# opas-lab/olearning-sim

Hardware: AMD Instinct MI355X
Metric: virtual clients/sec (simulated FL rounds, FedAvg CNN) (higher is better)
Workload: dtype bfloat16; 1 GPU; model=resnet18, preset=resnet-10k, clients_total=1250, clients_per_gpu=1250, local_steps=2, local_batch=16, num_classes=100, parallelism=dp1, global_batch=20000

## Files before the change

olearning_sim_amd/engine/local_train.py:

```python

from __future__ import annotations

from typing import Dict, Optional

import torch

from ..models.base import ClientBatchedModel, Params
from ..ops import fused
from .client_manager import FlatParams, replicate_params
from .data import SyntheticFederatedData


class LocalTrainer:
    def __init__(self, model: ClientBatchedModel, master: FlatParams,
                 data: SyntheticFederatedData, lr: float, prox_mu: float,
                 local_steps: int, batch_size: int, dtype: torch.dtype,
                 report_loss: bool = True):
        self.report_loss = report_loss
        self.model = model
        self.master = master
        self.data = data
        self.lr = lr
        self.prox_mu = prox_mu
        self.local_steps = local_steps
        self.batch_size = batch_size
        self.dtype = dtype
        self._cast_flat: Optional[torch.Tensor] = None

    def begin_round(self) -> None:
        self._cast_flat = self.master.flat.to(self.dtype)

    def _cast_params(self) -> Params:
        assert self._cast_flat is not None, "begin_round() not called"
        return self.master.views_of(self._cast_flat)

    def train_chunk(self, client_ids: torch.Tensor, weights: torch.Tensor,
                    round_idx: int, delta_flat: torch.Tensor,
                    wsum: Optional[float] = None) -> Dict[str, float]:
        C = int(client_ids.numel())
        cast = self._cast_params()
        params = replicate_params(cast, C)
        plist = list(params.values())
        glist = [cast[k] for k in params]
        last_loss = 0.0
        for step in range(self.local_steps):
            x, y = self.data.batch(client_ids, round_idx, step,
                                   self.batch_size, self.dtype)
            loss = self.model.loss(params, x, y)
            grads = torch.autograd.grad(loss * C, plist, allow_unused=True)
            with torch.no_grad():
                live = [(p, g) for p, g in zip(plist, grads) if g is not None]
                fused.fused_sgd_update(
                    [p for p, _ in live], [g for _, g in live],
                    lr=self.lr, mu=self.prox_mu,
                    global_params=[cast[k] for k, g in
                                   zip(params, grads) if g is not None])
            if self.report_loss and step == self.local_steps - 1:
                last_loss = float(loss.detach())
            del grads
        with torch.no_grad():
            delta_views = list(self.master.views_of(delta_flat).values())
            fused.weighted_delta_accum(
                delta_views, [p.detach() for p in plist], glist, weights,
                wsum=wsum if wsum is not None else float(weights.sum()))
        return {"loss": last_loss, "clients": C}
```

olearning_sim_amd/models/resnet.py:

```python

from __future__ import annotations

from typing import Optional

import torch

from .base import (ClientBatchedModel, Params, binit, kaiming,
                   blinear, bconv2d)

_STAGES = (64, 128, 256, 512)
_GN_GROUPS = 8


class ResNet18(ClientBatchedModel):
    name = "resnet18"
    num_classes = 100
    act_elems_per_sample = 1_600_000
    input_shape = (3, 32, 32)

    def __init__(self, num_classes: int = 100, in_ch: int = 3,
                 width_mult: float = 1.0):
        self.num_classes = num_classes
        self.in_ch = in_ch
        self.widths = [int(w * width_mult) for w in _STAGES]
        self.input_shape = (in_ch, 32, 32)

    def init_global(self, device="cpu", dtype=torch.float32,
                    generator: Optional[torch.Generator] = None) -> Params:
        g = generator
        p: Params = {}

        def conv(name, oc, ic, k):
            p[f"{name}.w"] = kaiming((oc, ic, k, k), ic * k * k, device, dtype, g)

        def gn(name, ch):
            p[f"{name}.g"] = torch.ones(ch, device=device, dtype=dtype)
            p[f"{name}.b"] = torch.zeros(ch, device=device, dtype=dtype)

        w = self.widths
        conv("stem", w[0], self.in_ch, 3)
        gn("stem.gn", w[0])
        in_c = w[0]
        for s, out_c in enumerate(w):
            for blk in range(2):
                pre = f"s{s}.b{blk}"
                ic = in_c if blk == 0 else out_c
                conv(f"{pre}.c1", out_c, ic, 3)
                gn(f"{pre}.gn1", out_c)
                conv(f"{pre}.c2", out_c, out_c, 3)
                gn(f"{pre}.gn2", out_c)
                if blk == 0 and (ic != out_c or s > 0):
                    conv(f"{pre}.down", out_c, ic, 1)
                    gn(f"{pre}.gndown", out_c)
            in_c = out_c
        p["fc.w"] = binit((w[3], self.num_classes), w[3], device, dtype, g)
        p["fc.b"] = binit((self.num_classes,), w[3], device, dtype, g)
        return p

    def _block(self, params: Params, x: torch.Tensor, C: int, pre: str,
               stride: int, has_down: bool) -> torch.Tensor:
        from ..ops.fused import groupnorm_act
        h = bconv2d(x, params[f"{pre}.c1.w"], C, stride=stride, padding=1)
        h = groupnorm_act(h, C, _GN_GROUPS, params[f"{pre}.gn1.g"],
                          params[f"{pre}.gn1.b"], relu=True)
        h = bconv2d(h, params[f"{pre}.c2.w"], C, stride=1, padding=1)
        if has_down:
            sc = bconv2d(x, params[f"{pre}.down.w"], C, stride=stride)
            sc = groupnorm_act(sc, C, _GN_GROUPS, params[f"{pre}.gndown.g"],
                               params[f"{pre}.gndown.b"])
        else:
            sc = x
        return groupnorm_act(h, C, _GN_GROUPS, params[f"{pre}.gn2.g"],
                             params[f"{pre}.gn2.b"], res=sc, relu=True)

    def _block_cbf(self, params: Params, x: torch.Tensor, x_pad, C: int,
                   pre: str, stride: int, has_down: bool,
                   pad_out: bool = True):
        from ..ops.conv import conv3x3_gn_relu, client_conv1x1
        from ..ops.fused import groupnorm_act
        h, h_pad = conv3x3_gn_relu(x, x_pad, params[f"{pre}.c1.w"], stride,
                                   C, _GN_GROUPS, params[f"{pre}.gn1.g"],
                                   params[f"{pre}.gn1.b"])
        if has_down:
            sc = client_conv1x1(x, params[f"{pre}.down.w"], stride,
                                x_pad=x_pad)
            sc = groupnorm_act(sc, C, _GN_GROUPS, params[f"{pre}.gndown.g"],
                               params[f"{pre}.gndown.b"])
            sc_pad = None
        else:
            sc, sc_pad = x, x_pad
        return conv3x3_gn_relu(h, h_pad, params[f"{pre}.c2.w"], 1, C,
                               _GN_GROUPS, params[f"{pre}.gn2.g"],
                               params[f"{pre}.gn2.b"], res=sc,
                               res_pad=sc_pad, pad_out=pad_out)

    def forward_cbf(self, params: Params, x: torch.Tensor) -> torch.Tensor:
        from ..ops.conv import client_conv3x3
        from ..ops.fused import groupnorm_relu_pad
        C, B = x.shape[0], x.shape[1]
        h = x.permute(0, 2, 1, 3, 4).contiguous()
        h = client_conv3x3(h, params["stem.w"], 1)
        h, h_pad = groupnorm_relu_pad(h, C, _GN_GROUPS, params["stem.gn.g"],
                                      params["stem.gn.b"])
        for s in range(4):
            stride = 1 if s == 0 else 2
            h, h_pad = self._block_cbf(params, h, h_pad, C, f"s{s}.b0",
                                       stride, s > 0)
            h, h_pad = self._block_cbf(params, h, h_pad, C, f"s{s}.b1", 1,
                                       False, pad_out=s < 3)
        h = h.mean(dim=(3, 4)).permute(0, 2, 1)
        return blinear(h, params["fc.w"], params["fc.b"])

    def forward(self, params: Params, x: torch.Tensor) -> torch.Tensor:
        from ..ops.fused import groupnorm_act
        import os
        if x.is_cuda and x.dtype == torch.bfloat16 and \
                os.environ.get("OLSIM_CONV", "custom") == "custom":
            from ..ops.fused import hip_ops_available
            if hip_ops_available():
                return self.forward_cbf(params, x)
        C, B = x.shape[0], x.shape[1]
        h = x.permute(1, 0, 2, 3, 4).reshape(B, C * self.in_ch, 32, 32)
        h = bconv2d(h, params["stem.w"], C, stride=1, padding=1)
        h = groupnorm_act(h, C, _GN_GROUPS, params["stem.gn.g"],
                          params["stem.gn.b"], relu=True)
        for s in range(4):
            stride = 1 if s == 0 else 2
            has_down = s > 0
            h = self._block(params, h, C, f"s{s}.b0", stride, has_down)
            h = self._block(params, h, C, f"s{s}.b1", 1, False)
        h = h.mean(dim=(2, 3)).reshape(B, C, self.widths[3]).permute(1, 0, 2)
        return blinear(h, params["fc.w"], params["fc.b"])
```

olearning_sim_amd/ops/build.py:

```python

from __future__ import annotations

import os
import shutil
import sys


def build(verbose: bool = True) -> str:
    os.environ.setdefault("PYTORCH_ROCM_ARCH", "gfx950")
    here = os.path.dirname(os.path.abspath(__file__))
    csrc = os.path.join(here, "csrc")
    build_dir = os.path.join(here, "_build")
    os.makedirs(build_dir, exist_ok=True)
    sources = [os.path.join(csrc, f) for f in
               ("bindings.cpp", "fused_update.hip", "aggregate.hip",
                "cross_entropy.hip", "groupnorm.hip", "client_conv.hip",
                "client_conv2.hip", "client_conv5.hip", "pool2x2.hip", "transpose.hip", "layernorm.hip", "pad2d.hip",
               "replicate.hip")]
    from torch.utils.cpp_extension import load
    mod_path = load(
        name="olsim_hip_ops",
        sources=sources,
        extra_cflags=["-O3"],
        extra_cuda_cflags=["-O3"],
        build_directory=build_dir,
        is_python_module=False,
        verbose=verbose,
    )
    built = os.path.join(build_dir, "olsim_hip_ops.so")
    target = os.path.join(here, "_hip_ops.so")
    if os.path.exists(built):
        shutil.copy2(built, target)
    return target


if __name__ == "__main__":
    path = build()
    print(f"built: {path}", file=sys.stderr)
```

olearning_sim_amd/ops/conv.py:

```python

from __future__ import annotations

import torch
import torch.nn.functional as F

from .fused import load_hip_ops


def _cpu_conv3x3(x: torch.Tensor, w: torch.Tensor, stride: int) -> torch.Tensor:
    C, IC, B, H, W = x.shape
    OC = w.shape[1]
    xg = x.permute(2, 0, 1, 3, 4).reshape(B, C * IC, H, W)
    wf = w.reshape(C * OC, IC, 3, 3)
    y = F.conv2d(xg, wf, stride=stride, padding=1, groups=C)
    OH, OW = y.shape[-2:]
    return y.reshape(B, C, OC, OH, OW).permute(1, 2, 0, 3, 4).contiguous()


class _Conv3x3Fn(torch.autograd.Function):
    @staticmethod
    def forward(ctx, x, w, stride):
        ops = load_hip_ops(required=True)
        y = ops.conv3x3_fwd(x, w, stride)
        ctx.save_for_backward(x, w)
        ctx.stride = stride
        return y

    @staticmethod
    def backward(ctx, dy):
        x, w = ctx.saved_tensors
        ops = load_hip_ops(required=True)
        dy = dy.contiguous()
        dx = dw = None
        if ctx.needs_input_grad[0]:
            dx = ops.conv3x3_dgrad(dy, w, x.shape[3], x.shape[4], ctx.stride)
        if ctx.needs_input_grad[1]:
            dw = ops.conv3x3_wgrad(x, dy, ctx.stride)
        return dx, dw, None


def _pad(x: torch.Tensor, pad: int) -> torch.Tensor:
    import os
    if (x.is_cuda and x.dtype == torch.bfloat16 and x.shape[-1] % 2 == 0
            and os.environ.get("OLSIM_PAD", "") != "torch"):
        ops = load_hip_ops()
        if ops is not None:
            return ops.pad2d(x.contiguous(), pad)
    return F.pad(x, (pad, pad, pad, pad))


class _Conv3x3PadFn(torch.autograd.Function):

    @staticmethod
    def forward(ctx, x, w, stride):
        ops = load_hip_ops(required=True)
        x_pad = _pad(x, 1)
        y = ops.conv3x3_fwd_p(x_pad, w, stride)
        ctx.save_for_backward(x_pad, w)
        ctx.stride = stride
        return y

    @staticmethod
    def backward(ctx, dy):
        x_pad, w = ctx.saved_tensors
        ops = load_hip_ops(required=True)
        dy = dy.contiguous()
        dx = dw = None
        H, W = x_pad.shape[3] - 2, x_pad.shape[4] - 2
        if ctx.needs_input_grad[0]:
            dy_pad = _pad(dy, 1)
            dx = ops.conv3x3_dgrad_p(dy_pad, w, H, W, ctx.stride)
        if ctx.needs_input_grad[1]:
            dw = ops.conv3x3_wgrad_p(x_pad, dy, ctx.stride)
        return dx, dw, None


class _Conv3x3GnPadFn(torch.autograd.Function):

    @staticmethod
    def forward(ctx, x, x_pad, w, res, res_pad, gamma, beta, clients,
                groups, eps, stride, pad_out):
        from .fused import _interior, _res_arg
        ops = load_hip_ops(required=True)
        h = ops.conv3x3_fwd_p(x_pad, w, stride)
        y, mask, mean, rstd = ops.groupnorm_fwd_pad(
            h, _res_arg(h, res, res_pad), gamma, beta, clients, groups, eps,
            pad_out)
        ctx.save_for_backward(x_pad, w, h, mask, mean, rstd, gamma)
        ctx.meta = (clients, groups, res is not None, stride)
        ctx.set_materialize_grads(False)
        if not pad_out:
            return y, None
        ctx.mark_non_differentiable(y)
        return _interior(y), y

    @staticmethod
    def backward(ctx, dy, _dy_pad):
        x_pad, w, h, mask, mean, rstd, gamma = ctx.saved_tensors
        clients, groups, has_res, stride = ctx.meta
        if dy is None:
            return (None,) * 12
        ops = load_hip_ops(required=True)
        need_dx = ctx.needs_input_grad[0]
        dh, dh_pad, dres, dgamma, dbeta = ops.groupnorm_bwd_pad(
            h, mask, dy, mean, rstd, gamma, clients, groups, has_res,
            need_dx)
        H, W = x_pad.shape[3] - 2, x_pad.shape[4] - 2
        dx = dw = None
        if need_dx:
            dx = ops.conv3x3_dgrad_p(dh_pad, w, H, W, stride)
        if ctx.needs_input_grad[2]:
            dw = ops.conv3x3_wgrad_p(x_pad, dh, stride)
        return (dx, None, dw, dres if has_res else None, None,
                dgamma.to(gamma.dtype), dbeta.to(gamma.dtype),
                None, None, None, None, None)


def conv3x3_gn_relu(x: torch.Tensor, x_pad, w: torch.Tensor, stride: int,
                    clients: int, groups: int, gamma: torch.Tensor,
                    beta: torch.Tensor, res=None, res_pad=None,
                    pad_out: bool = True, eps: float = 1e-5):
    from .fused import gn_pad_shape_ok, groupnorm_act
    if x.is_cuda and x.dtype == torch.bfloat16:
        ops = load_hip_ops(required=True)
        OH = (x.shape[3] + stride - 1) // stride
        OW = (x.shape[4] + stride - 1) // stride
        if _v6_ok(ops, x, w, stride) and gn_pad_shape_ok(w.shape[1], groups,
                                                         OH, OW):
            if x_pad is None:
                x_pad = _pad(x, 1)
            return _Conv3x3GnPadFn.apply(
                x, x_pad, w.contiguous(), res, res_pad, gamma.contiguous(),
                beta.contiguous(), clients, groups, eps, stride, pad_out)
    h = client_conv3x3(x, w, stride)
    return groupnorm_act(h, clients, groups, gamma, beta, res=res,
                         relu=True, eps=eps), None


def _v6_ok(ops, x: torch.Tensor, w: torch.Tensor, stride: int) -> bool:
    import os
    if os.environ.get("OLSIM_CONV_V", "") == "5":
        return False
    C, IC, B, H, W = x.shape
    return bool(ops.conv3x3_v6_ok(IC, w.shape[1], B, H, W, stride))


def client_conv3x3(x: torch.Tensor, w: torch.Tensor,
                   stride: int = 1) -> torch.Tensor:
    if x.is_cuda and x.dtype == torch.bfloat16:
        ops = load_hip_ops(required=True)
        if _v6_ok(ops, x, w, stride):
            return _Conv3x3PadFn.apply(x.contiguous(), w.contiguous(), stride)
        return _Conv3x3Fn.apply(x.contiguous(), w.contiguous(), stride)
    return _cpu_conv3x3(x, w, stride)



_NTAB_CACHE: dict = {}


def _ntab(B: int, OH: int, OW: int, H: int, W: int,
          device: torch.device) -> torch.Tensor:
    key = (B, OH, OW, H, W, str(device))
    t = _NTAB_CACHE.get(key)
    if t is None:
        n = torch.arange(B * OH * OW, dtype=torch.int64)
        b, q = n // (OH * OW), n % (OH * OW)
        t = (b * H * W + (q // OW) * W + (q % OW)).to(torch.int32).to(device)
        if len(_NTAB_CACHE) < 64:
            _NTAB_CACHE[key] = t
    return t


def _cpu_conv5x5(x, w, b, relu):
    C, IC, B, H, W = x.shape
    OC = w.shape[1]
    xg = x.permute(2, 0, 1, 3, 4).reshape(B, C * IC, H, W)
    y = F.conv2d(xg, w.reshape(C * OC, IC, 5, 5), b.reshape(C * OC),
                 groups=C)
    OH, OW = y.shape[-2:]
    y = y.reshape(B, C, OC, OH, OW).permute(1, 2, 0, 3, 4).contiguous()
    return F.relu(y) if relu else y


class _Conv5x5Fn(torch.autograd.Function):

    @staticmethod
    def forward(ctx, x, w, b, relu):
        ops = load_hip_ops(required=True)
        C, IC, B, H, W = x.shape
        nt = _ntab(B, H - 4, W - 4, H, W, x.device)
        y = ops.conv5x5_fwd(x, w, b, nt, relu)
        ctx.save_for_backward(x, w, y)
# ... 115 lines not shown
```

olearning_sim_amd/ops/csrc/bindings.cpp:

```cpp

#include <torch/extension.h>
#include <ATen/cuda/CUDAContext.h>
#include <hip/hip_runtime.h>

#include "ols_ops.h"

namespace {

int dtype_code(const at::Tensor& t) {
  switch (t.scalar_type()) {
    case at::kFloat: return 0;
    case at::kBFloat16: return 1;
    case at::kHalf: return 2;
    default:
      TORCH_CHECK(false, "olsim_hip: unsupported dtype ", t.scalar_type());
  }
}

void fused_sgd_update_flat(at::Tensor buf, at::Tensor grad,
                           at::Tensor global_flat, at::Tensor offsets,
                           int64_t clients, double lr, double mu) {
  TORCH_CHECK(buf.is_cuda() && buf.is_contiguous(), "buf must be GPU+contig");
  TORCH_CHECK(grad.sizes() == buf.sizes() && grad.scalar_type() == buf.scalar_type());
  const bool prox = mu != 0.0 && global_flat.numel() > 0;
// ... 187 lines not shown
                  d.B, d.H, d.W, (int)stride,
                  at::cuda::getCurrentCUDAStream().stream());
  return y;
}

at::Tensor conv3x3_dgrad(at::Tensor dy, at::Tensor w, int64_t H, int64_t W,
                         int64_t stride) {
  const ConvDims d = conv_dims(3, {}, 0, dy, 0, w, H, W, stride);
  auto dx = at::empty({d.C, d.IC, d.B, d.H, d.W}, dy.options());
  ols_conv3x3_dgrad(dy.data_ptr(), w.data_ptr(), dx.data_ptr(), d.C, d.IC,
                    d.OC, d.B, d.H, d.W, (int)stride,
                    at::cuda::getCurrentCUDAStream().stream());
  return dx;
}

at::Tensor conv3x3_wgrad(at::Tensor x, at::Tensor dy, int64_t stride) {
  const ConvDims d = conv_dims(3, x, 0, dy, 0, {}, 0, 0, stride);
  auto dw = at::empty({d.C, d.OC, d.IC, 3, 3}, x.options());
  ols_conv3x3_wgrad(x.data_ptr(), dy.data_ptr(), dw.data_ptr(), d.C, d.IC,
                    d.OC, d.B, d.H, d.W, (int)stride,
                    at::cuda::getCurrentCUDAStream().stream());
  return dw;
}


bool conv3x3_v6_ok(int64_t IC, int64_t OC, int64_t B, int64_t H, int64_t W,
                   int64_t stride) {
  return ols_conv3x3_v6_ok((int)IC, (int)OC, (int)B, (int)H, (int)W,
                           (int)stride) != 0;
}

std::string conv3x3_route(std::string dir, int64_t IC, int64_t OC, int64_t B,
                          int64_t H, int64_t W, int64_t stride) {
  int d = dir == "fwd" ? 0 : dir == "dgrad" ? 1 : dir == "wgrad" ? 2 : -1;
  TORCH_CHECK(d >= 0, "conv3x3_route: dir must be fwd, dgrad or wgrad");
  TORCH_CHECK(stride == 1 || stride == 2, "conv3x3_route: stride 1 or 2");
  return ols_conv3x3_route(d, (int)IC, (int)OC, (int)B, (int)H, (int)W,
                           (int)stride);
}

std::string conv3x3_staging(std::string dir, int64_t IC, int64_t OC,
                            int64_t B, int64_t H, int64_t W, int64_t stride) {
  int d = dir == "fwd" ? 0 : dir == "dgrad" ? 1 : dir == "wgrad" ? 2 : -1;
  TORCH_CHECK(d >= 0, "conv3x3_staging: dir must be fwd, dgrad or wgrad");
  TORCH_CHECK(stride == 1 || stride == 2, "conv3x3_staging: stride 1 or 2");
  return ols_conv3x3_staging(d, (int)IC, (int)OC, (int)B, (int)H, (int)W,
                             (int)stride);
}

void check_v6(const ConvDims& d, int64_t stride) {
  TORCH_CHECK(ols_conv3x3_v6_ok(d.IC, d.OC, d.B, d.H, d.W, (int)stride),
              "shape unsupported by the v6 conv path");
}

at::Tensor conv3x3_fwd_p(at::Tensor xp, at::Tensor w, int64_t stride) {
  const ConvDims d = conv_dims(3, xp, 1, {}, 0, w, 0, 0, stride);
  check_v6(d, stride);
  auto y = at::empty({d.C, d.OC, d.B, d.OH, d.OW}, xp.options());
  ols_conv3x3_fwd_p(xp.data_ptr(), w.data_ptr(), y.data_ptr(), d.C, d.IC,
                    d.OC, d.B, d.H, d.W, (int)stride,
                    at::cuda::getCurrentCUDAStream().stream());
  return y;
}

at::Tensor conv3x3_dgrad_p(at::Tensor dyp, at::Tensor w, int64_t H, int64_t W,
                           int64_t stride) {
  const ConvDims d = conv_dims(3, {}, 0, dyp, 1, w, H, W, stride);
  check_v6(d, stride);
  auto dx = at::empty({d.C, d.IC, d.B, d.H, d.W}, dyp.options());
  ols_conv3x3_dgrad_p(dyp.data_ptr(), w.data_ptr(), dx.data_ptr(), d.C, d.IC,
                      d.OC, d.B, d.H, d.W, (int)stride,
                      at::cuda::getCurrentCUDAStream().stream());
  return dx;
}

at::Tensor conv3x3_wgrad_p(at::Tensor xp, at::Tensor dy, int64_t stride) {
  const ConvDims d = conv_dims(3, xp, 1, dy, 0, {}, 0, 0, stride);
  check_v6(d, stride);
  auto dw = at::empty({d.C, d.OC, d.IC, 3, 3}, xp.options());
  ols_conv3x3_wgrad_p(xp.data_ptr(), dy.data_ptr(), dw.data_ptr(), d.C, d.IC,
                      d.OC, d.B, d.H, d.W, (int)stride,
                      at::cuda::getCurrentCUDAStream().stream());
  return dw;
}


std::string conv5x5_route(std::string dir, int64_t IC, int64_t OC, int64_t H,
                          int64_t W) {
  int d = dir == "fwd" ? 0 : dir == "dgrad" ? 1 : dir == "wgrad" ? 2 : -1;
  TORCH_CHECK(d >= 0, "conv5x5_route: dir must be fwd, dgrad or wgrad");
  int r = ols_conv5x5_route(d, (int)IC, (int)OC, (int)H, (int)W);
  return r == 0 ? "direct" : r == 1 ? "mfma" : "two_stage";
}

void check_ntab(const at::Tensor& ntab, const at::Tensor& on, int64_t n) {
  TORCH_CHECK(ntab.is_cuda() && ntab.device() == on.device() &&
                  ntab.scalar_type() == at::kInt && ntab.is_contiguous() &&
                  ntab.numel() == n,
              "conv5x5: ntab must be ", n, " contiguous int32 on the GPU");
}

at::Tensor conv5x5_fwd(at::Tensor x, at::Tensor w, at::Tensor bias,
                       at::Tensor ntab, bool relu) {
  const ConvDims d = conv_dims(5, x, 0, {}, 0, w, 0, 0, 1);
  TORCH_CHECK(d.OC <= 16);
  check_ntab(ntab, x, (int64_t)d.B * d.OH * d.OW);
  TORCH_CHECK(bias.is_cuda() && bias.scalar_type() == at::kBFloat16 &&
              bias.numel() == (int64_t)d.C * d.OC);
  auto y = at::empty({d.C, d.OC, d.B, d.OH, d.OW}, x.options());
  ols_conv5x5_fwd(x.data_ptr(), w.data_ptr(), bias.contiguous().data_ptr(),
                  y.data_ptr(), ntab.data_ptr<int>(), d.C, d.IC, d.OC, d.B,
                  d.H, d.W, relu ? 1 : 0,
                  at::cuda::getCurrentCUDAStream().stream());
  return y;
}

at::Tensor conv5x5_dgrad(at::Tensor dyp, at::Tensor w, at::Tensor ntab,
                         int64_t H, int64_t W) {
  const ConvDims d = conv_dims(5, {}, 0, dyp, 4, w, H, W, 1);
  TORCH_CHECK(d.IC <= 16);
  check_ntab(ntab, dyp, (int64_t)d.B * d.H * d.W);
  auto dx = at::empty({d.C, d.IC, d.B, d.H, d.W}, dyp.options());
  ols_conv5x5_dgrad(dyp.data_ptr(), w.data_ptr(), dx.data_ptr(),
                    ntab.data_ptr<int>(), d.C, d.IC, d.OC, d.B, d.H, d.W,
                    at::cuda::getCurrentCUDAStream().stream());
  return dx;
}

at::Tensor conv5x5_wgrad(at::Tensor x, at::Tensor dy, at::Tensor ntab) {
  const ConvDims d = conv_dims(5, x, 0, dy, 0, {}, 0, 0, 1);
  const int64_t nq = (int64_t)d.B * d.OH * d.OW;
  TORCH_CHECK(d.OC <= 16 && nq % 32 == 0);
  check_ntab(ntab, x, nq);
  auto dw = at::empty({d.C, d.OC, d.IC, 5, 5}, x.options());
  at::Tensor part;
  float* partp = nullptr;
  if (ols_conv5x5_route(2, d.IC, d.OC, d.H, d.W) == 2) {
    part = at::empty({(int64_t)d.C * d.B * d.OC * d.IC * 25},
                     x.options().dtype(at::kFloat));
    partp = part.data_ptr<float>();
  }
  ols_conv5x5_wgrad(x.data_ptr(), dy.data_ptr(), dw.data_ptr(), partp,
                    ntab.data_ptr<int>(), d.C, d.IC, d.OC, d.B, d.H, d.W,
                    at::cuda::getCurrentCUDAStream().stream());
  return dw;
}


std::tuple<at::Tensor, at::Tensor> pool2x2_fwd(at::Tensor x) {
  TORCH_CHECK(x.is_cuda() && x.is_contiguous() && x.dim() >= 2);
  int H = x.size(-2), W = x.size(-1);
  TORCH_CHECK(H % 2 == 0 && W % 2 == 0);
  int64_t planes = x.numel() / ((int64_t)H * W);
  auto sizes = x.sizes().vec();
  sizes[sizes.size() - 2] = H / 2;
  sizes[sizes.size() - 1] = W / 2;
  auto y = at::empty(sizes, x.options());
  auto arg = at::empty(sizes, x.options().dtype(at::kByte));
  int dt = x.scalar_type() == at::kBFloat16 ? 1 : 0;
  ols_pool2x2_fwd(x.data_ptr(), y.data_ptr(),
                  (unsigned char*)arg.data_ptr(), planes, H / 2, W / 2, dt,
                  at::cuda::getCurrentCUDAStream().stream());
  return {y, arg};
}

at::Tensor pool2x2_bwd(at::Tensor dy, at::Tensor arg) {
// ... 195 lines not shown
              y.scalar_type() == at::kLong);
  int64_t rows = y.numel(), batch = x.size(0), n = x.size(1);
  TORCH_CHECK(rows % batch == 0);
  auto out = at::empty({rows, n}, x.options().dtype(at::kBFloat16));
  ols_synth_batch(x.data_ptr<float>(), y.data_ptr<int64_t>(),
                  out.data_ptr(), rows, batch, n, (float)s, (float)t,
                  at::cuda::getCurrentCUDAStream().stream());
  return out;
}


at::Tensor relu_mask(at::Tensor dy, at::Tensor y) {
  TORCH_CHECK(dy.is_cuda() && dy.is_contiguous() && y.is_contiguous());
  TORCH_CHECK(dy.sizes() == y.sizes() && dy.scalar_type() == y.scalar_type());
  TORCH_CHECK(dy.numel() % 8 == 0);
  TORCH_CHECK(dy.scalar_type() == at::kBFloat16 ||
              dy.scalar_type() == at::kFloat);
  auto out = at::empty_like(dy);
  int dt = dy.scalar_type() == at::kBFloat16 ? 1 : 0;
  ols_relu_mask(dy.data_ptr(), y.data_ptr(), out.data_ptr(), dy.numel(), dt,
                at::cuda::getCurrentCUDAStream().stream());
  return out;
}


at::Tensor pad2d(at::Tensor x, int64_t pad) {
  TORCH_CHECK(x.is_cuda() && x.is_contiguous() && x.dim() >= 2);
  TORCH_CHECK(x.scalar_type() == at::kBFloat16 ||
              x.scalar_type() == at::kHalf);
  int H = x.size(-2), W = x.size(-1);
  TORCH_CHECK(W % 2 == 0 && pad >= 1);
  int64_t planes = x.numel() / ((int64_t)H * W);
  auto sizes = x.sizes().vec();
  sizes[sizes.size() - 2] = H + 2 * pad;
  sizes[sizes.size() - 1] = W + 2 * pad;
  auto y = at::empty(sizes, x.options());
  int dt = x.scalar_type() == at::kBFloat16 ? 1 : 2;
  ols_pad2d(x.data_ptr(), y.data_ptr(), planes, H, W, (int)pad, dt,
            at::cuda::getCurrentCUDAStream().stream());
  return y;
}


at::Tensor transpose2d(at::Tensor x) {
  TORCH_CHECK(x.is_cuda() && x.is_contiguous() && x.dim() == 3);
  TORCH_CHECK(x.scalar_type() == at::kBFloat16 ||
              x.scalar_type() == at::kFloat);
  int64_t B = x.size(0);
  int M = x.size(1), N = x.size(2);
  TORCH_CHECK(B <= 65535, "transpose2d: batch ", B, " exceeds 65535");
  auto y = at::empty({B, (int64_t)N, (int64_t)M}, x.options());
  int dt = x.scalar_type() == at::kBFloat16 ? 1 : 0;
  ols_transpose2d(x.data_ptr(), y.data_ptr(), B, M, N, dt,
                  at::cuda::getCurrentCUDAStream().stream());
  return y;
}

}

TORCH_LIBRARY(olsim_hip, m) {
  m.def("fused_sgd_update_flat(Tensor(a!) buf, Tensor grad, Tensor global_flat, "
        "Tensor offsets, int clients, float lr, float mu) -> ()");
  m.def("weighted_delta_accum_flat(Tensor(a!) delta, Tensor buf, "
        "Tensor global_flat, Tensor weights, Tensor offsets, int clients, float wsum) -> ()");
  m.def("cross_entropy_fwd_bwd(Tensor logits, Tensor labels) -> (Tensor, Tensor)");
  m.def("groupnorm_fwd(Tensor x, Tensor res, Tensor gamma, Tensor beta, "
        "int clients, int groups, float eps, bool relu) -> (Tensor, Tensor, Tensor)");
  m.def("groupnorm_bwd(Tensor x, Tensor y, Tensor dy, Tensor mean, "
        "Tensor rstd, Tensor gamma, int clients, int groups, bool has_res, "
        "bool relu) -> (Tensor, Tensor, Tensor, Tensor)");
  m.def("mfma_selftest(Tensor A, Tensor B) -> Tensor");
  m.def("conv3x3_fwd(Tensor x, Tensor w, int stride) -> Tensor");
  m.def("conv3x3_dgrad(Tensor dy, Tensor w, int H, int W, int stride) -> Tensor");
  m.def("conv3x3_wgrad(Tensor x, Tensor dy, int stride) -> Tensor");
  m.def("conv3x3_v6_ok(int IC, int OC, int B, int H, int W, int stride) -> bool",
        &conv3x3_v6_ok);
  m.def("conv3x3_route(str dir, int IC, int OC, int B, int H, int W, "
        "int stride) -> str", &conv3x3_route);
  m.def("conv3x3_staging(str dir, int IC, int OC, int B, int H, int W, "
        "int stride) -> str", &conv3x3_staging);
  m.def("conv3x3_fwd_p(Tensor xp, Tensor w, int stride) -> Tensor");
  m.def("conv3x3_dgrad_p(Tensor dyp, Tensor w, int H, int W, int stride) -> Tensor");
  m.def("conv3x3_wgrad_p(Tensor xp, Tensor dy, int stride) -> Tensor");
  m.def("conv5x5_route(str dir, int IC, int OC, int H, int W) -> str",
        &conv5x5_route);
  m.def("conv5x5_fwd(Tensor x, Tensor w, Tensor bias, Tensor ntab, bool relu) -> Tensor");
  m.def("conv5x5_dgrad(Tensor dyp, Tensor w, Tensor ntab, int H, int W) -> Tensor");
  m.def("conv5x5_wgrad(Tensor x, Tensor dy, Tensor ntab) -> Tensor");
  m.def("pool2x2_fwd(Tensor x) -> (Tensor, Tensor)");
  m.def("pool2x2_bwd(Tensor dy, Tensor arg) -> Tensor");
  m.def("transpose2d(Tensor x) -> Tensor");
  m.def("pad2d(Tensor x, int pad) -> Tensor");
  m.def("relu_mask(Tensor dy, Tensor y) -> Tensor");
  m.def("replicate(Tensor src, int clients) -> Tensor");
  m.def("subsample2(Tensor x) -> Tensor");
  m.def("subsample2_bwd(Tensor dy, int H, int W) -> Tensor");
  m.def("subsample2_p(Tensor xp) -> Tensor");
  m.def("gn_pad_ok(int ch, int groups, int H, int W) -> bool", &gn_pad_ok);
  m.def("groupnorm_fwd_pad(Tensor x, Tensor res, Tensor gamma, Tensor beta, "
        "int clients, int groups, float eps, bool pad_out) -> "
        "(Tensor, Tensor, Tensor, Tensor)");
  m.def("groupnorm_bwd_pad(Tensor x, Tensor mask, Tensor dy, Tensor mean, "
        "Tensor rstd, Tensor gamma, int clients, int groups, bool has_res, "
        "bool want_pad) -> (Tensor, Tensor, Tensor, Tensor, Tensor)");
  m.def("synth_batch(Tensor x, Tensor y, float s, float t) -> Tensor");
  m.def("layernorm_fwd(Tensor x, Tensor gamma, Tensor beta, float eps) -> (Tensor, Tensor, Tensor)");
  m.def("layernorm_bwd(Tensor x, Tensor dy, Tensor gamma, Tensor mean, Tensor rstd) -> (Tensor, Tensor, Tensor)");
}

TORCH_LIBRARY_IMPL(olsim_hip, CUDA, m) {
  m.impl("fused_sgd_update_flat", &fused_sgd_update_flat);
  m.impl("weighted_delta_accum_flat", &weighted_delta_accum_flat);
  m.impl("cross_entropy_fwd_bwd", &cross_entropy_fwd_bwd);
  m.impl("groupnorm_fwd", &groupnorm_fwd);
  m.impl("groupnorm_bwd", &groupnorm_bwd);
  m.impl("mfma_selftest", &mfma_selftest);
  m.impl("conv3x3_fwd", &conv3x3_fwd);
  m.impl("conv3x3_dgrad", &conv3x3_dgrad);
  m.impl("conv3x3_wgrad", &conv3x3_wgrad);
  m.impl("conv3x3_fwd_p", &conv3x3_fwd_p);
  m.impl("conv3x3_dgrad_p", &conv3x3_dgrad_p);
  m.impl("conv3x3_wgrad_p", &conv3x3_wgrad_p);
  m.impl("conv5x5_fwd", &conv5x5_fwd);
  m.impl("conv5x5_dgrad", &conv5x5_dgrad);
  m.impl("conv5x5_wgrad", &conv5x5_wgrad);
  m.impl("pool2x2_fwd", &pool2x2_fwd);
  m.impl("pool2x2_bwd", &pool2x2_bwd);
  m.impl("transpose2d", &transpose2d);
  m.impl("pad2d", &pad2d);
  m.impl("relu_mask", &relu_mask);
  m.impl("replicate", &replicate);
  m.impl("subsample2", &subsample2);
  m.impl("subsample2_bwd", &subsample2_bwd);
  m.impl("subsample2_p", &subsample2_p);
  m.impl("groupnorm_fwd_pad", &groupnorm_fwd_pad);
  m.impl("groupnorm_bwd_pad", &groupnorm_bwd_pad);
  m.impl("synth_batch", &synth_batch);
  m.impl("layernorm_fwd", &layernorm_fwd);
  m.impl("layernorm_bwd", &layernorm_bwd);
}
```

olearning_sim_amd/ops/csrc/ols_ops.h:

```cpp
#pragma once

#include <hip/hip_runtime.h>
#include <cstdint>

#define MAX_CG 128

extern "C" void ols_fused_sgd_update_flat(
    void* buf, const void* grad, const void* master, const int64_t* offs,
    int nblocks, int64_t clients, int64_t total, float lr, float mu,
    int dtype, hipStream_t stream);

extern "C" void ols_weighted_delta_accum_flat(
    float* delta, const void* buf, const void* master, const float* weights,
    const int64_t* offs, int nblocks, int64_t clients, int64_t pglobal,
    float wsum, int dtype, hipStream_t stream);

extern "C" void ols_cross_entropy_fwd_bwd(
    const void* logits, const int64_t* labels, float* loss, void* dlogits,
    int64_t nrows, int64_t K, float inv_n, int dtype, hipStream_t stream);

extern "C" void ols_groupnorm_fwd(const void* x, const void* res, void* y,
                                  float* mean, float* rstd, const void* gamma,
                                  const void* beta, int B, int C, int ch,
                                  int G, int HW, float eps, bool relu,
                                  int layout, int dtype, hipStream_t stream);

extern "C" void ols_mfma_selftest(const void* A, const void* B, float* D,
                                  hipStream_t stream);

extern "C" void ols_conv3x3_fwd(const void* x, const void* w, void* y, int C,
                                int IC, int OC, int B, int H, int W,
                                int stride, hipStream_t stream);
extern "C" void ols_conv3x3_dgrad(const void* dy, const void* w, void* dx,
                                  int C, int IC, int OC, int B, int H, int W,
                                  int stride, hipStream_t stream);
extern "C" void ols_conv3x3_wgrad(const void* x, const void* dy, void* dw,
                                  int C, int IC, int OC, int B, int H, int W,
                                  int stride, hipStream_t stream);

extern "C" int ols_conv3x3_v6_ok(int IC, int OC, int B, int H, int W,
                                 int stride);
extern "C" const char* ols_conv3x3_route(int dir, int IC, int OC, int B,
                                         int H, int W, int stride);
extern "C" const char* ols_conv3x3_staging(int dir, int IC, int OC, int B,
                                           int H, int W, int stride);
extern "C" void ols_conv3x3_fwd_p(const void* xp, const void* w, void* y,
                                  int C, int IC, int OC, int B, int H, int W,
                                  int stride, hipStream_t stream);
extern "C" void ols_conv3x3_dgrad_p(const void* dyp, const void* w, void* dx,
                                    int C, int IC, int OC, int B, int H,
                                    int W, int stride, hipStream_t stream);
extern "C" void ols_conv3x3_wgrad_p(const void* xp, const void* dy, void* dw,
                                    int C, int IC, int OC, int B, int H,
                                    int W, int stride, hipStream_t stream);

extern "C" void ols_conv5x5_fwd(const void* x, const void* w, const void* b,
                                void* y, const int* ntab, int C, int IC,
                                int OC, int B, int H, int W, int relu,
                                hipStream_t stream);
extern "C" void ols_conv5x5_dgrad(const void* dyp, const void* w, void* dx,
                                  const int* ntab, int C, int IC, int OC,
                                  int B, int H, int W, hipStream_t stream);
extern "C" int ols_conv5x5_route(int dir, int IC, int OC, int H, int W);
extern "C" void ols_conv5x5_wgrad(const void* x, const void* dy, void* dw,
                                  float* part, const int* ntab, int C,
                                  int IC, int OC, int B, int H, int W,
                                  hipStream_t stream);

extern "C" void ols_pool2x2_fwd(const void* x, void* y, unsigned char* arg,
                                int64_t planes, int OH, int OW, int dtype,
                                hipStream_t stream);
extern "C" void ols_pool2x2_bwd(const void* dy, const unsigned char* arg,
                                void* dx, int64_t planes, int OH, int OW,
                                int dtype, hipStream_t stream);

extern "C" void ols_subsample2_fwd(const void* x, void* y, int64_t planes,
                                   int OH, int OW, int dtype,
                                   hipStream_t stream);
extern "C" void ols_subsample2_bwd(const void* dy, void* dx, int64_t planes,
                                   int H, int W, int dtype,
                                   hipStream_t stream);

extern "C" void ols_transpose2d(const void* in, void* out, int64_t B, int M,
                                int N, int dtype, hipStream_t stream);

extern "C" void ols_pad2d(const void* in, void* out, int64_t planes, int H,
                          int W, int pad, int dtype, hipStream_t stream);

extern "C" void ols_replicate(const void* src, void* dst, int64_t clients,
                              int64_t n, int dtype, hipStream_t stream);

extern "C" void ols_synth_batch(const float* x, const int64_t* y, void* out,
                                int64_t rows, int64_t batch, int64_t n,
                                float s, float t, hipStream_t stream);

extern "C" void ols_relu_mask(const void* dy, const void* y, void* out,
                              int64_t n, int dtype, hipStream_t stream);

extern "C" void ols_layernorm_fwd(const void* x, const void* gamma,
                                  const void* beta, void* y, float* mean,
                                  float* rstd, int64_t rows, int H,
                                  int64_t rows_per_client, float eps,
                                  int dtype, hipStream_t stream);
extern "C" void ols_layernorm_bwd(const void* x, const void* dy,
                                  const void* gamma, const float* mean,
                                  const float* rstd, void* dx, float* dgamma,
                                  float* dbeta, int64_t rows, int H,
                                  int64_t rows_per_client, int dtype,
                                  hipStream_t stream);

extern "C" void ols_groupnorm_bwd(const void* x, const void* y,
                                  const void* dy, void* dx, void* dres,
                                  const float* mean, const float* rstd,
                                  const void* gamma, float* dgamma,
                                  float* dbeta, int B, int C, int ch, int G,
                                  int HW, bool relu, int layout, int dtype,
                                  hipStream_t stream);

extern "C" int ols_gn_pad_ok(int ch, int G, int H, int W);
extern "C" void ols_groupnorm_fwd_pad(
    const void* x, const void* res, int res_mode, void* y, uint32_t* mask,
    float* mean, float* rstd, const void* gamma, const void* beta, int B,
    int C, int ch, int G, int H, int W, float eps, bool pad_out,
    hipStream_t stream);
extern "C" void ols_groupnorm_bwd_pad(
    const void* x, const uint32_t* mask, const void* dy, void* dx,
    void* dx_pad, void* dres, const float* mean, const float* rstd,
    const void* gamma, float* dgamma, float* dbeta, int B, int C, int ch,
    int G, int H, int W, hipStream_t stream);
extern "C" void ols_subsample2p_fwd(const void* xp, void* y, int64_t planes,
                                    int OH, int OW, int dtype,
                                    hipStream_t stream);
```

olearning_sim_amd/ops/fused.py:

```python

from __future__ import annotations

import os
from typing import Optional, Sequence

import torch

_HIP_OPS = None
_HIP_OPS_TRIED = False

_SO_NAME = "_hip_ops.so"


def _so_path() -> str:
    return os.path.join(os.path.dirname(os.path.abspath(__file__)), _SO_NAME)


def load_hip_ops(required: bool = False):
    global _HIP_OPS, _HIP_OPS_TRIED
    if _HIP_OPS is not None:
        return _HIP_OPS
    if _HIP_OPS_TRIED and not required:
        return None
    _HIP_OPS_TRIED = True
    path = _so_path()
    if os.path.exists(path):
        torch.ops.load_library(path)
        _HIP_OPS = torch.ops.olsim_hip
        return _HIP_OPS
    if required:
        raise RuntimeError(
            f"olearning_sim_amd HIP extension missing: {path} not built. "
            f"Run `python -m olearning_sim_amd.ops.build` (hipcc, gfx950).")
    return None


def hip_ops_available() -> bool:
    return load_hip_ops() is not None


_OFFS_CACHE = {}
_EMPTY_OFFS = None


def _cached_offsets(n: int, device) -> torch.Tensor:
    key = (n, str(device))
    t = _OFFS_CACHE.get(key)
    if t is None:
        t = torch.tensor([0, n], dtype=torch.int64, device=device)
        _OFFS_CACHE[key] = t
    return t


def _gpu_ops(t: torch.Tensor):
    if t.is_cuda:
        return load_hip_ops(required=True)
    return None


def fused_sgd_update(params: Sequence[torch.Tensor],
                     grads: Sequence[torch.Tensor],
                     lr: float,
                     mu: float = 0.0,
                     global_params: Optional[Sequence[torch.Tensor]] = None) -> None:
    if not params:
        return
    if params[0].is_cuda:
        for i, (w, g) in enumerate(zip(params, grads)):
            n = w[0].numel() if w.dim() > 1 else w.numel()
            gl = (global_params[i].reshape(-1) if (global_params is not None
                                                  and mu != 0.0)
                  else torch.empty(0, dtype=w.dtype, device=w.device))
            offs = (_cached_offsets(n, w.device) if mu != 0.0
                    else _cached_offsets(0, w.device)[:0])
            fused_sgd_update_flat(w.reshape(-1), g.reshape(-1), gl,
                                  w.shape[0], lr, mu, offs)
        return
    with torch.no_grad():
        for i, (w, g) in enumerate(zip(params, grads)):
            upd = g
            if mu != 0.0 and global_params is not None:
                upd = g + mu * (w - global_params[i].to(w.dtype))
            w.add_(upd, alpha=-lr)


def weighted_delta_accum(delta: Sequence[torch.Tensor],
                         client_params: Sequence[torch.Tensor],
                         global_params: Sequence[torch.Tensor],
                         weights: torch.Tensor,
                         wsum: Optional[float] = None) -> None:
    if not delta:
        return
    if client_params[0].is_cuda:
        if wsum is None:
            wsum = float(weights.sum())
        for dl, cw, gw in zip(delta, client_params, global_params):
            offs = _cached_offsets(gw.numel(), cw.device)
            weighted_delta_accum_flat(dl.reshape(-1), cw.reshape(-1),
                                      gw.reshape(-1), weights, cw.shape[0],
                                      offs, wsum)
        return
    with torch.no_grad():
        for dl, cw, gw in zip(delta, client_params, global_params):
            diff = cw.float() - gw.float().unsqueeze(0)
            shape = [-1] + [1] * (cw.dim() - 1)
            dl.add_((diff * weights.view(shape)).sum(dim=0))


def apply_aggregate(global_params: Sequence[torch.Tensor],
                    delta: Sequence[torch.Tensor],
                    total_weight: float) -> None:
    if total_weight == 0:
        return
    with torch.no_grad():
        inv = 1.0 / float(total_weight)
        torch._foreach_add_([g for g in global_params],
                            [d for d in delta], alpha=inv)



def fused_sgd_update_flat(buf: torch.Tensor, grad: torch.Tensor,
                          global_flat: torch.Tensor, clients: int,
                          lr: float, mu: float,
                          offsets: Optional[torch.Tensor] = None) -> None:
    if buf.is_cuda:
        ops = load_hip_ops(required=True)
        ops.fused_sgd_update_flat(
            buf, grad,
            global_flat if mu != 0.0 else torch.empty(0, dtype=buf.dtype, device=buf.device),
            offsets if (mu != 0.0 and offsets is not None) else
            torch.empty(0, dtype=torch.int64, device=buf.device),
            int(clients), float(lr), float(mu))
        return
    with torch.no_grad():
        if mu == 0.0 or offsets is None:
            buf.add_(grad, alpha=-lr)
            return
        offs = offsets.tolist()
        for b in range(len(offs) - 1):
            g0, g1 = offs[b], offs[b + 1]
            n = g1 - g0
            blk = buf[clients * g0:clients * g1].view(clients, n)
            gblk = grad[clients * g0:clients * g1].view(clients, n)
            prox = blk - global_flat[g0:g1].unsqueeze(0)
            blk.add_(gblk + mu * prox, alpha=-lr)


def weighted_delta_accum_flat(delta: torch.Tensor, buf: torch.Tensor,
                              global_flat: torch.Tensor,
                              weights: torch.Tensor, clients: int,
                              offsets: Optional[torch.Tensor] = None,
# ... 196 lines not shown
```

Measured before the change: 1962 clients/s.

## Cache flipped-transposed conv3x3 weights for dgrad via forward kernel, fused with SGD

Adds a kernel that flips and transposes 3x3 conv weights so that the data-gradient can be computed by the faster forward conv kernel instead of the dedicated dgrad kernel. The transposed weights are built once per chunk from the master weights and replicated per client. The SGD step for those weights is fused with regenerating the transposed copy, so later local steps reuse it without a separate flip. This costs extra memory for a per-client transposed weight copy. Validity depends on tracking the tensor version so a stale copy is never used.

```diff
diff --git a/olearning_sim_amd/engine/local_train.py b/olearning_sim_amd/engine/local_train.py
--- a/olearning_sim_amd/engine/local_train.py
+++ b/olearning_sim_amd/engine/local_train.py
@@ -34,6 +34,22 @@
         assert self._cast_flat is not None, "begin_round() not called"
         return self.master.views_of(self._cast_flat)
 
+    def _attach_master_wt(self, cast: Params, params: Params, C: int) -> None:
+        import os
+        wanted = getattr(self.model, "dgrad_wt_params", None)
+        if (wanted is None or self.dtype != torch.bfloat16
+                or not self._cast_flat.is_cuda
+                or os.environ.get("OLSIM_DGRAD_WT", "1") == "repack"):
+            return
+        from ..ops.conv import attach_wt, dgrad_wt_ok
+        ops = fused.load_hip_ops(required=True)
+        for k, (H, W) in wanted(cast).items():
+            OC, IC = cast[k].shape[0], cast[k].shape[1]
+            if not dgrad_wt_ok(ops, OC, IC, self.batch_size, H, W):
+                continue
+            wt0 = ops.conv3x3_wflip(cast[k].detach().clone()[None])[0]
+            attach_wt(params[k], ops.replicate(wt0, C))
+
     def train_chunk(self, client_ids: torch.Tensor, weights: torch.Tensor,
                     round_idx: int, delta_flat: torch.Tensor,
                     wsum: Optional[float] = None) -> Dict[str, float]:
@@ -42,6 +58,7 @@
         params = replicate_params(cast, C)
         plist = list(params.values())
         glist = [cast[k] for k in params]
+        self._attach_master_wt(cast, params, C)
         last_loss = 0.0
         for step in range(self.local_steps):
             x, y = self.data.batch(client_ids, round_idx, step,
@@ -54,7 +71,8 @@
                     [p for p, _ in live], [g for _, g in live],
                     lr=self.lr, mu=self.prox_mu,
                     global_params=[cast[k] for k, g in
-                                   zip(params, grads) if g is not None])
+                                   zip(params, grads) if g is not None],
+                    keep_wt=step < self.local_steps - 1)
             if self.report_loss and step == self.local_steps - 1:
                 last_loss = float(loss.detach())
             del grads
diff --git a/olearning_sim_amd/models/resnet.py b/olearning_sim_amd/models/resnet.py
--- a/olearning_sim_amd/models/resnet.py
+++ b/olearning_sim_amd/models/resnet.py
@@ -1,6 +1,7 @@
 
 from __future__ import annotations
 
+import os
 from typing import Optional
 
 import torch
@@ -94,6 +95,18 @@
                                params[f"{pre}.gn2.b"], res=sc,
                                res_pad=sc_pad, pad_out=pad_out)
 
+    def dgrad_wt_params(self, params: Params):
+        if os.environ.get("OLSIM_CONV", "custom") != "custom":
+            return {}
+        planes = {}
+        for s in range(4):
+            for blk in range(2):
+                for cv in ("c1", "c2"):
+                    if s > 0 and blk == 0 and cv == "c1":
+                        continue
+                    planes[f"s{s}.b{blk}.{cv}.w"] = (32 >> s, 32 >> s)
+        return planes
+
     def forward_cbf(self, params: Params, x: torch.Tensor) -> torch.Tensor:
         from ..ops.conv import client_conv3x3
         from ..ops.fused import groupnorm_relu_pad
@@ -113,7 +126,6 @@
 
     def forward(self, params: Params, x: torch.Tensor) -> torch.Tensor:
         from ..ops.fused import groupnorm_act
-        import os
         if x.is_cuda and x.dtype == torch.bfloat16 and \
                 os.environ.get("OLSIM_CONV", "custom") == "custom":
             from ..ops.fused import hip_ops_available
diff --git a/olearning_sim_amd/ops/build.py b/olearning_sim_amd/ops/build.py
--- a/olearning_sim_amd/ops/build.py
+++ b/olearning_sim_amd/ops/build.py
@@ -15,7 +15,7 @@
     sources = [os.path.join(csrc, f) for f in
                ("bindings.cpp", "fused_update.hip", "aggregate.hip",
                 "cross_entropy.hip", "groupnorm.hip", "client_conv.hip",
-                "client_conv2.hip", "client_conv5.hip", "pool2x2.hip", "transpose.hip", "layernorm.hip", "pad2d.hip",
+                "client_conv2.hip", "conv3_wflip.hip", "client_conv5.hip", "pool2x2.hip", "transpose.hip", "layernorm.hip", "pad2d.hip",
                "replicate.hip")]
     from torch.utils.cpp_extension import load
     mod_path = load(
diff --git a/olearning_sim_amd/ops/conv.py b/olearning_sim_amd/ops/conv.py
--- a/olearning_sim_amd/ops/conv.py
+++ b/olearning_sim_amd/ops/conv.py
@@ -49,6 +49,42 @@
     return F.pad(x, (pad, pad, pad, pad))
 
 
+def attach_wt(w: torch.Tensor, wt: torch.Tensor) -> None:
+    w._olsim_wt = [wt, w._version]
+
+
+def drop_wt(w: torch.Tensor) -> None:
+    held = getattr(w, "_olsim_wt", None)
+    if held is not None:
+        held[0] = None
+        w._olsim_wt = None
+
+
+def _live_wt(held, w: torch.Tensor):
+    if held is None or held[0] is None or held[1] != w._version:
+        return None
+    return held[0]
+
+
+def dgrad_wt_ok(ops, OC: int, IC: int, B: int, H: int, W: int,
+                stride: int = 1) -> bool:
+    import os
+    return (stride == 1 and os.environ.get("OLSIM_DGRAD_WT", "1") != "0"
+            and "OLSIM_CONV_DW64" not in os.environ
+            and bool(ops.conv3x3_v6_ok(OC, IC, B, H, W, 1)))
+
+
+def _dgrad_p(ops, dy_pad: torch.Tensor, w: torch.Tensor, H: int, W: int,
+             stride: int, held=None) -> torch.Tensor:
+    if dgrad_wt_ok(ops, w.shape[1], w.shape[2], dy_pad.shape[2], H, W,
+                   stride):
+        wt = _live_wt(held, w)
+        if wt is None:
+            wt = ops.conv3x3_wflip(w)
+        return ops.conv3x3_fwd_p(dy_pad, wt, 1)
+    return ops.conv3x3_dgrad_p(dy_pad, w, H, W, stride)
+
+
 class _Conv3x3PadFn(torch.autograd.Function):
 
     @staticmethod
@@ -58,6 +94,7 @@
         y = ops.conv3x3_fwd_p(x_pad, w, stride)
         ctx.save_for_backward(x_pad, w)
         ctx.stride = stride
+        ctx.wt = getattr(w, "_olsim_wt", None)
         return y
 
     @staticmethod
@@ -69,7 +106,7 @@
         H, W = x_pad.shape[3] - 2, x_pad.shape[4] - 2
         if ctx.needs_input_grad[0]:
             dy_pad = _pad(dy, 1)
-            dx = ops.conv3x3_dgrad_p(dy_pad, w, H, W, ctx.stride)
+            dx = _dgrad_p(ops, dy_pad, w, H, W, ctx.stride, ctx.wt)
         if ctx.needs_input_grad[1]:
             dw = ops.conv3x3_wgrad_p(x_pad, dy, ctx.stride)
         return dx, dw, None
@@ -88,6 +125,7 @@
             pad_out)
         ctx.save_for_backward(x_pad, w, h, mask, mean, rstd, gamma)
         ctx.meta = (clients, groups, res is not None, stride)
+        ctx.wt = getattr(w, "_olsim_wt", None)
         ctx.set_materialize_grads(False)
         if not pad_out:
             return y, None
@@ -108,7 +146,7 @@
         H, W = x_pad.shape[3] - 2, x_pad.shape[4] - 2
         dx = dw = None
         if need_dx:
-            dx = ops.conv3x3_dgrad_p(dh_pad, w, H, W, stride)
+            dx = _dgrad_p(ops, dh_pad, w, H, W, stride, ctx.wt)
         if ctx.needs_input_grad[2]:
             dw = ops.conv3x3_wgrad_p(x_pad, dh, stride)
         return (dx, None, dw, dres if has_res else None, None,
diff --git a/olearning_sim_amd/ops/csrc/bindings.cpp b/olearning_sim_amd/ops/csrc/bindings.cpp
--- a/olearning_sim_amd/ops/csrc/bindings.cpp
+++ b/olearning_sim_amd/ops/csrc/bindings.cpp
@@ -293,6 +293,64 @@
                       d.OC, d.B, d.H, d.W, (int)stride,
                       at::cuda::getCurrentCUDAStream().stream());
   return dw;
+}
+
+
+struct WflipDims {
+  int C, OC, IC;
+};
+
+WflipDims wflip_dims(const at::Tensor& w, const at::Tensor& g,
+                     const at::Tensor& wt) {
+  TORCH_CHECK(w.is_cuda() && w.is_contiguous() && w.dim() == 5 &&
+                  w.scalar_type() == at::kBFloat16 && w.size(3) == 3 &&
+                  w.size(4) == 3,
+              "conv3x3_wflip: w must be a contiguous bf16 [C, OC, IC, 3, 3] "
+              "GPU tensor, got ", w.scalar_type(), " ", w.sizes());
+  const int64_t C = w.size(0), OC = w.size(1), IC = w.size(2);
+  TORCH_CHECK(C > 0 && OC > 0 && IC > 0 && OC % 32 == 0 && IC % 32 == 0,
+              "conv3x3_wflip: OC and IC must be multiples of 32, got ",
+              w.sizes());
+  TORCH_CHECK(C * (OC / 32) * (IC / 32) <= INT32_MAX,
+              "conv3x3_wflip: too many tiles");
+  for (const at::Tensor* t : {&w, &g, &wt}) {
+    if (!t->defined()) continue;
+    TORCH_CHECK(t->is_cuda() && t->is_contiguous() &&
+                    t->scalar_type() == at::kBFloat16 &&
+                    t->device() == w.device() &&
+                    reinterpret_cast<uintptr_t>(t->data_ptr()) % 16 == 0,
+                "conv3x3_wflip: operands must be contiguous, 16-byte "
+                "aligned bf16 tensors on one GPU");
+  }
+  TORCH_CHECK(!g.defined() || g.sizes() == w.sizes(),
+              "sgd_conv3_wt: g is ", g.sizes(), ", expected ", w.sizes());
+  TORCH_CHECK(!wt.defined() ||
+                  wt.sizes() == at::IntArrayRef({C, IC, OC, 3, 3}),
+              "sgd_conv3_wt: wt is ", wt.sizes(), ", expected [", C, ", ",
+              IC, ", ", OC, ", 3, 3]");
+  return {(int)C, (int)OC, (int)IC};
+}
+
+at::Tensor conv3x3_wflip(at::Tensor w) {
+  const WflipDims d = wflip_dims(w, {}, {});
+  auto wt = at::empty({d.C, d.IC, d.OC, 3, 3}, w.options());
+  ols_conv3_wflip(w.data_ptr(), wt.data_ptr(), d.C, d.OC, d.IC,
+                  at::cuda::getCurrentCUDAStream().stream());
+  return wt;
+}
+
+void sgd_conv3_wt(at::Tensor w, at::Tensor g, at::Tensor wt, double lr) {
+  const WflipDims d = wflip_dims(w, g, wt);
+  const char* wtp = static_cast<const char*>(wt.data_ptr());
+  const int64_t nbytes = (int64_t)wt.numel() * 2;
+  for (const at::Tensor* t : {&w, &g}) {
+    const char* p = static_cast<const char*>(t->data_ptr());
+    TORCH_CHECK(p + nbytes <= wtp || wtp + nbytes <= p,
+                "sgd_conv3_wt: wt must not overlap w or g");
+  }
+  ols_sgd_conv3_wt(w.data_ptr(), g.data_ptr(), wt.data_ptr(), d.C, d.OC,
+                   d.IC, (float)lr,
+                   at::cuda::getCurrentCUDAStream().stream());
 }
 
 
@@ -654,6 +712,8 @@
   m.def("conv3x3_fwd_p(Tensor xp, Tensor w, int stride) -> Tensor");
   m.def("conv3x3_dgrad_p(Tensor dyp, Tensor w, int H, int W, int stride) -> Tensor");
   m.def("conv3x3_wgrad_p(Tensor xp, Tensor dy, int stride) -> Tensor");
+  m.def("conv3x3_wflip(Tensor w) -> Tensor");
+  m.def("sgd_conv3_wt(Tensor(a!) w, Tensor g, Tensor(b!) wt, float lr) -> ()");
   m.def("conv5x5_route(str dir, int IC, int OC, int H, int W) -> str",
         &conv5x5_route);
   m.def("conv5x5_fwd(Tensor x, Tensor w, Tensor bias, Tensor ntab, bool relu) -> Tensor");
@@ -693,6 +753,8 @@
   m.impl("conv3x3_fwd_p", &conv3x3_fwd_p);
   m.impl("conv3x3_dgrad_p", &conv3x3_dgrad_p);
   m.impl("conv3x3_wgrad_p", &conv3x3_wgrad_p);
+  m.impl("conv3x3_wflip", &conv3x3_wflip);
+  m.impl("sgd_conv3_wt", &sgd_conv3_wt);
   m.impl("conv5x5_fwd", &conv5x5_fwd);
   m.impl("conv5x5_dgrad", &conv5x5_dgrad);
   m.impl("conv5x5_wgrad", &conv5x5_wgrad);
diff --git a/olearning_sim_amd/ops/csrc/conv3_wflip.hip b/olearning_sim_amd/ops/csrc/conv3_wflip.hip
--- /dev/null
+++ b/olearning_sim_amd/ops/csrc/conv3_wflip.hip
@@ -0,0 +1,105 @@
+
+#include "common.h"
+#include "ols_ops.h"
+
+#define WF_TILE 32
+#define WF_ROW (WF_TILE * 9)
+#define WF_CHUNKS (WF_TILE * WF_ROW / 8)
+#define WF_THREADS 384
+#define WF_PASSES (WF_CHUNKS / WF_THREADS)
+
+static_assert(WF_CHUNKS % WF_THREADS == 0, "whole passes");
+
+__device__ __forceinline__ int64_t wf_row_off(int c, int R, int S, int r0,
+                                              int row, int s0) {
+  return (((int64_t)c * R + r0 + row) * S + s0) * 9;
+}
+
+__device__ __forceinline__ uint4 wf_gather(const ushort* lds, int ic, int j) {
+  int oc = (8 * j) / 9;
+  int r = 8 * j - 9 * oc;
+  Pack<ushort, 8> v;
+#pragma unroll
+  for (int e = 0; e < 8; ++e) {
+    v.v[e] = lds[oc * WF_ROW + ic * 9 + 8 - r];
+    if (++r == 9) { r = 0; ++oc; }
+  }
+  return __builtin_bit_cast(uint4, v);
+}
+
+template <bool SGD>
+__device__ __forceinline__ void wf_tile(
+    __hip_bfloat16* __restrict__ w, const __hip_bfloat16* __restrict__ g,
+    __hip_bfloat16* __restrict__ wt, int OC, int IC, float lr) {
+  __shared__ __attribute__((aligned(16))) ushort lds[WF_TILE * WF_ROW];
+  const int tiles_ic = IC / WF_TILE;
+  const int tiles = (OC / WF_TILE) * tiles_ic;
+  const int c = blockIdx.x / tiles;
+  const int tile = blockIdx.x - c * tiles;
+  const int oc0 = (tile / tiles_ic) * WF_TILE;
+  const int ic0 = (tile % tiles_ic) * WF_TILE;
+
+  uint4 in[WF_PASSES];
+#pragma unroll
+  for (int p = 0; p < WF_PASSES; ++p) {
+    const int i = threadIdx.x + p * WF_THREADS;
+    const int row = i / 36, col = i - row * 36;
+    const int64_t off = wf_row_off(c, OC, IC, oc0, row, ic0) + col * 8;
+    in[p] = *reinterpret_cast<const uint4*>(w + off);
+    if constexpr (SGD) {
+      using P8 = Pack<__hip_bfloat16, 8>;
+      P8 wv = __builtin_bit_cast(P8, in[p]);
+      const P8 gv = *reinterpret_cast<const P8*>(g + off);
+#pragma unroll
+      for (int k = 0; k < 8; ++k)
+        wv.v[k] = from_f32<__hip_bfloat16>(to_f32(wv.v[k]) -
+                                           lr * to_f32(gv.v[k]));
+      in[p] = __builtin_bit_cast(uint4, wv);
+      *reinterpret_cast<uint4*>(w + off) = in[p];
+    }
+  }
+#pragma unroll
+  for (int p = 0; p < WF_PASSES; ++p)
+    *reinterpret_cast<uint4*>(&lds[(threadIdx.x + p * WF_THREADS) * 8]) =
+        in[p];
+  __syncthreads();
+#pragma unroll
+  for (int p = 0; p < WF_PASSES; ++p) {
+    const int i = threadIdx.x + p * WF_THREADS;
+    const int ic = i / 36, j = i - ic * 36;
+    *reinterpret_cast<uint4*>(wt + wf_row_off(c, IC, OC, ic0, ic, oc0) +
+                              j * 8) = wf_gather(lds, ic, j);
+  }
+}
+
+__global__ __launch_bounds__(WF_THREADS) void k_conv3_wflip(
+    const __hip_bfloat16* __restrict__ w, __hip_bfloat16* __restrict__ wt,
+    int OC, int IC) {
+  wf_tile<false>(const_cast<__hip_bfloat16*>(w), nullptr, wt, OC, IC, 0.f);
+}
+
+__global__ __launch_bounds__(WF_THREADS) void k_sgd_conv3_wt(
+    __hip_bfloat16* __restrict__ w, const __hip_bfloat16* __restrict__ g,
+    __hip_bfloat16* __restrict__ wt, int OC, int IC, float lr) {
+  wf_tile<true>(w, g, wt, OC, IC, lr);
+}
+
+static inline unsigned wf_grid(int C, int OC, int IC) {
+  return (unsigned)((int64_t)C * (OC / WF_TILE) * (IC / WF_TILE));
+}
+
+extern "C" void ols_conv3_wflip(const void* w, void* wt, int C, int OC,
+                                int IC, hipStream_t stream) {
+  hipLaunchKernelGGL(k_conv3_wflip, dim3(wf_grid(C, OC, IC)),
+                     dim3(WF_THREADS), 0, stream, (const __hip_bfloat16*)w,
+                     (__hip_bfloat16*)wt, OC, IC);
+}
+
+extern "C" void ols_sgd_conv3_wt(void* w, const void* g, void* wt, int C,
+                                 int OC, int IC, float lr,
+                                 hipStream_t stream) {
+  hipLaunchKernelGGL(k_sgd_conv3_wt, dim3(wf_grid(C, OC, IC)),
+                     dim3(WF_THREADS), 0, stream, (__hip_bfloat16*)w,
+                     (const __hip_bfloat16*)g, (__hip_bfloat16*)wt, OC, IC,
+                     lr);
+}
diff --git a/olearning_sim_amd/ops/csrc/ols_ops.h b/olearning_sim_amd/ops/csrc/ols_ops.h
--- a/olearning_sim_amd/ops/csrc/ols_ops.h
+++ b/olearning_sim_amd/ops/csrc/ols_ops.h
@@ -53,6 +53,12 @@
 extern "C" void ols_conv3x3_wgrad_p(const void* xp, const void* dy, void* dw,
                                     int C, int IC, int OC, int B, int H,
                                     int W, int stride, hipStream_t stream);
+
+extern "C" void ols_conv3_wflip(const void* w, void* wt, int C, int OC,
+                                int IC, hipStream_t stream);
+extern "C" void ols_sgd_conv3_wt(void* w, const void* g, void* wt, int C,
+                                 int OC, int IC, float lr,
+                                 hipStream_t stream);
 
 extern "C" void ols_conv5x5_fwd(const void* x, const void* w, const void* b,
                                 void* y, const int* ntab, int C, int IC,
diff --git a/olearning_sim_amd/ops/fused.py b/olearning_sim_amd/ops/fused.py
--- a/olearning_sim_amd/ops/fused.py
+++ b/olearning_sim_amd/ops/fused.py
@@ -58,15 +58,30 @@
     return None
 
 
+def _wt_update_ok(w: torch.Tensor, g: torch.Tensor) -> bool:
+    return all(t.dtype == torch.bfloat16 and t.is_contiguous()
+               and t.data_ptr() % 16 == 0 for t in (w, g))
+
+
 def fused_sgd_update(params: Sequence[torch.Tensor],
                      grads: Sequence[torch.Tensor],
                      lr: float,
                      mu: float = 0.0,
-                     global_params: Optional[Sequence[torch.Tensor]] = None) -> None:
+                     global_params: Optional[Sequence[torch.Tensor]] = None,
+                     keep_wt: bool = False) -> None:
     if not params:
         return
     if params[0].is_cuda:
+        from .conv import _live_wt, attach_wt, drop_wt
         for i, (w, g) in enumerate(zip(params, grads)):
+            held = getattr(w, "_olsim_wt", None)
+            if held is not None:
+                wt = _live_wt(held, w) if keep_wt and mu == 0.0 else None
+                drop_wt(w)
+                if wt is not None and _wt_update_ok(w, g):
+                    load_hip_ops(required=True).sgd_conv3_wt(w, g, wt, lr)
+                    attach_wt(w, wt)
+                    continue
             n = w[0].numel() if w.dim() > 1 else w.numel()
             gl = (global_params[i].reshape(-1) if (global_params is not None
                                                   and mu != 0.0)
```

New measurement: 2079 clients/s, median of 6. +6.0%, better.
